# bnbowman/pbccs

Hardware: AMD Instinct MI355X
Metric: CCS ZMWs/sec (and GCUPS) at 1/2/4/8 MI355X vs host-CPU ccs (higher is better)
Workload: dtype f64

## Files before the change

### pbccs_amd/csrc/arrow_kernels.hip

```cpp
#include "arrow_device.hpp"
#include "arrow_kernels.hpp"
#include "arrow_score_device.hpp"
#include "coop_chain.hpp"

#include <climits>

namespace pbccs {

__device__ __forceinline__ LaneBand scratch_band(const FillScratch& F, int g, int l, int which)
{
    const long long gm = 2LL * g + which;
    LaneBand m;
    m.range = F.range + gm * F.capCols * 64 + l;
    m.off = F.off + gm * F.capCols * 64 + l;
    m.ls = F.ls + gm * F.capCols * 64 + l;
    m.val = F.val + gm * F.capSlots * 64 + l;
    m.cap = F.capSlots;
    return m;
}

__global__ void __launch_bounds__(64) k_fill(DevBatch B, FillScratch F, const int* __restrict__ reads, int n)
{
    const int t = blockIdx.x * blockDim.x + threadIdx.x;
    if (t >= n) return;
// ... 280 lines not shown
            cnt = (p == 0) ? 8 : 6 + (cur != prev ? 1 : 0);
        }
        int incl = cnt;
        for (int d = 1; d < 64; d <<= 1) {
            const int y = __shfl_up(incl, d, 64);
            if (lane >= d) incl += y;
        }
        if (lane == 63) waveSums[wid] = incl;
        __syncthreads();
        int waveOff = 0;
        for (int w = 0; w < wid; ++w) waveOff += waveSums[w];
        const int excl = carry + waveOff + incl - cnt;
        if (p < L) {
            po[p] = excl;
            int k = excl;
            for (int x = 0; x < 4; ++x)
                if (base_char(x) != cur) out[k++] = mut_code(p, kSub, x);
            for (int x = 0; x < 4; ++x)
                if (base_char(x) != prev) out[k++] = mut_code(p, kIns, x);
            if (cur != prev) out[k++] = mut_code(p, kDel, 0);
        }
        __syncthreads();
        if (threadIdx.x == 255) carry = excl + cnt;
        __syncthreads();
    }
    if (threadIdx.x == 0) po[L] = carry;
}

__device__ __forceinline__ bool read_scores(int ts, int te, int type, int ms, int me)
{
    if (type == kIns) return ts <= me && ms <= te;
    return ts < me && ms < te;
}

struct MidGeom {
    int b0, e0, b1, e1;
    int lb, le;
};

__device__ __forceinline__ MidGeom middle_geometry(const Band& a, const Band& b, int sc, int bc)
{
    MidGeom g;
    const int2 r0 = a.range[sc - 1], r1 = a.range[sc], r2 = a.range[sc + 1], r3 = a.range[sc + 2];
    g.b0 = min(min(r1.x, r0.x), r2.x);
    g.e0 = max(max(r1.y, r0.y), r2.y);
    g.b1 = min(min(r2.x, r1.x), r3.x);
    g.e1 = max(max(r2.y, r1.y), r3.y);
    const int2 q0 = b.range[bc], q1 = b.range[bc + 1];
    g.lb = min(min(g.b0, g.b1), min(q0.x, q1.x));
    g.le = max(max(g.e0, g.e1), max(q0.y, q1.y));
    return g;
}

__device__ __forceinline__ double score_middle(const ScoreCtx& S, int sc, int bc, const MidGeom& g,
                                               const double* __restrict__ av, int2 ar,
                                               const double* __restrict__ bv, int2 br,
                                               const char* __restrict__ rdp, TaskStat& st)
{
    const int I = S.I;
    char t0, t1, t2, t3;
    int x0, x1, x2, x3;
    S.tv.At(sc - 2, t0, x0);
    S.tv.At(sc - 1, t1, x1);
    S.tv.At(sc, t2, x2);
    S.tv.At(sc + 1, t3, x3);
    (void)t0;
    const double* P0 = S.P.P(sc > 1 ? x0 : kCtxZero);
    const double* P1 = S.P.P(x1);
    const double* P2 = S.P.P(x2);
    const double pM0 = P0[kM], pD0 = P0[kD], cB0 = P1[kB], cS0 = P1[kS3];
    const double pM1 = P1[kM], pD1 = P1[kD], cB1 = P2[kB], cS1 = P2[kS3];
    const double lM = P2[kM], lD = P2[kD];
    const double pn = S.P.prNot, p3 = S.P.prThird;

#define PB_ALPHA(i) (((i) >= ar.x && (i) < ar.y) ? av[(i)] : 0.0)
#define PB_BETA(i) (((i) >= br.x && (i) < br.y) ? bv[-(i)] : 0.0)
#define PB_CELL(out, i, rb, curB, nxtB, pM, pD, cB, cS, pd, pl, rawPrev)                    \
    {                                                                                     \
        const double em_ = ((rb) == (curB)) ? pn : p3;                                    \
        double s_ = ((i) > 0) ? (((i) < I) ? (pd) * (pM) * em_ : 0.0) : (rawPrev);        \
        if ((i) > 1 && (i) < I) s_ = s_ + (rawPrev) * (((nxtB) == (rb)) ? (cB) : (cS));   \
        if ((i) != I) s_ = s_ + (pl) * (pD);                                              \
        out = s_;                                                                         \
    }

    double C0 = 0.0;
    {
        double aD = PB_ALPHA(g.b0 - 1), raw = 0.0;
        for (int i = g.b0; i < g.e0; ++i) {
            const double aL = PB_ALPHA(i);
            const char rb = rdp[i - 1];
            double v;
            PB_CELL(v, i, rb, t1, t2, pM0, pD0, cB0, cS0, aD, aL, raw);
            raw = v;
            if (C0 < v) C0 = v;
            aD = aL;
        }
    }
    const bool s0 = (C0 != 0.0 && C0 != 1.0);
    const int u0 = min(g.b0, g.b1), u1 = max(g.e0, g.e1);
    double C1 = 0.0;
    {
        double aD = PB_ALPHA(u0 - 1), raw0 = 0.0, raw1 = 0.0, sc0p = 0.0;
        for (int i = u0; i < u1; ++i) {
            const double aL = PB_ALPHA(i);
            const char rb = rdp[i - 1];
            double v0 = 0.0, v1 = 0.0, sc0 = 0.0;
            if (i >= g.b0 && i < g.e0) {
                PB_CELL(v0, i, rb, t1, t2, pM0, pD0, cB0, cS0, aD, aL, raw0);
                sc0 = s0 ? v0 / C0 : v0;
            }
            if (i >= g.b1 && i < g.e1) {
                PB_CELL(v1, i, rb, t2, t3, pM1, pD1, cB1, cS1, sc0p, sc0, raw1);
                if (C1 < v1) C1 = v1;
            }
            raw0 = v0;
            raw1 = v1;
            sc0p = sc0;
            aD = aL;
        }
    }
    const bool s1 = (C1 != 0.0 && C1 != 1.0);
    double v = 0.0;
    {
        double aD = PB_ALPHA(g.lb - 1), raw0 = 0.0, raw1 = 0.0, sc0p = 0.0;
        double bH = PB_BETA(g.lb);
        for (int i = g.lb; i < g.le; ++i) {
            const double aL = PB_ALPHA(i);
            const double bN = PB_BETA(i + 1);
            const char rb = (i >= 1) ? rdp[i - 1] : (char)0;
            double v0 = 0.0, v1 = 0.0, sc0 = 0.0, sc1 = 0.0;
            if (i >= g.b0 && i < g.e0) {
                PB_CELL(v0, i, rb, t1, t2, pM0, pD0, cB0, cS0, aD, aL, raw0);
                sc0 = s0 ? v0 / C0 : v0;
            }
            if (i >= g.b1 && i < g.e1) {
                PB_CELL(v1, i, rb, t2, t3, pM1, pD1, cB1, cS1, sc0p, sc0, raw1);
                sc1 = s1 ? v1 / C1 : v1;
            }
            if (i < I) {
                const double mprob = lM * ((rdp[i] == t3) ? pn : p3);
                v = v + sc1 * mprob * bN;
            }
            v = v + sc1 * lD * bH;
            raw0 = v0;
            raw1 = v1;
            sc0p = sc0;
            aD = aL;
            bH = bN;
        }
    }
#undef PB_CELL
#undef PB_BETA
#undef PB_ALPHA
    const double E = (0.0 + (s0 ? log(C0) : 0.0)) + (s1 ? log(C1) : 0.0);
    st.cells += (unsigned long long)(max(0, g.e0 - g.b0) + max(0, g.e1 - g.b1) + max(0, g.le - g.lb));
    st.bytes += 8ull * (unsigned long long)(max(0, ar.y - ar.x) + max(0, br.y - br.x)) + 16ull * 6ull;
    return ((log(v) + E) + S.bSuf[bc]) + S.aPre[sc];
}

struct Oriented {
    int os, oe, ld, type;
};

__device__ __forceinline__ Oriented setup_score(const DevBatch& B, int r, int code, ScoreCtx& S)
{
    const int z = B.rZmw[r];
    const int L = B.zLen[z];
    const int ts = B.rTs[r], te = B.rTe[r];
    Oriented o;
    o.type = mut_type(code);
    const int pos = mut_pos(code);
    const int base = mut_base(code);
    const int mEnd = (o.type == kIns) ? pos : pos + 1;
    o.ld = (o.type == kIns) ? 1 : (o.type == kDel ? -1 : 0);
    S.B = &B;
    S.P = params_for(B, z);
    S.rd = B.seqPool + B.rSeqOff[r];
    S.I = B.rLen[r];
    S.Jorig = te - ts;
    S.a = band_alpha(B, r);
    S.b = band_beta(B, r);
    const long long cbase = B.rColBase[r];
    S.aPre = B.aPre + cbase;
    S.bSuf = B.bSuf + cbase;
    S.tv = window_view(B, r);
    if (B.rStrand[r] == kFwd) {
        S.tv.vm = make_virtual(S.tv.T, L, o.type, pos, base_char(base));
        o.os = pos - ts;
        o.oe = mEnd - ts;
    } else {
        S.tv.vm = make_virtual(S.tv.T, L, o.type, L - mEnd, base_char(complement_index(base)));
        o.os = te - mEnd;
        o.oe = te - pos;
    }
    return o;
}

__device__ double score_edge(const ScoreCtx& S, const Oriented& o, const ScoreScratch& scratch, TaskStat& st)
{
    const int J = S.Jorig;
    const bool atBegin = o.os < 3;
    const bool atEnd = o.oe > (J + 1) - 1 - 2;
    if (!atBegin && atEnd) {
        const int sc = o.os - 1;
        const int n = S.tv.Length() - sc + 1;
        return extend_alpha_score<TplView, kMaxExtCols>(S, sc, n, false, 0, 0, st);
    }
    if (atBegin && !atEnd) return extend_beta_score<TplView, kMaxExtCols>(S, o.oe, o.ld, st);
    if (!atBegin && !atEnd) {
        const int sc = (o.type == kDel) ? o.os - 1 : o.os;
        return extend_alpha_score<TplView, kMaxExtCols>(S, sc, 2, true, 1 + o.oe, 1 + o.oe + o.ld, st);
    }
    const int Jv = S.tv.Length();
    const long long ncol = Jv + 1;
    const long long need = ncol * (long long)(S.I + 1) + 4 * ncol + 16;
    const unsigned long long at = atomicAdd(scratch.top, (unsigned long long)need);
    if (at + need > scratch.cap) {
        atomicOr(scratch.overflow, 1);
        return __longlong_as_double(0x7ff8000000000001LL);
    }
    double* base0 = scratch.pool + at;
    Band m;
    m.ls = base0;
    m.range = reinterpret_cast<int2*>(base0 + ncol);
    m.off = reinterpret_cast<int*>(base0 + 2 * ncol);
    m.val = base0 + 4 * ncol;
    m.cap = ncol * (long long)(S.I + 1);
    const long long u = fill_alpha(S.tv, S.rd, S.I, m, (const Band*)nullptr, false, S.P);
    st.cells += (unsigned long long)max(0LL, u);
    st.bytes += 8ull * (unsigned long long)max(0LL, u) + 16ull * (unsigned long long)ncol;
    return log(alpha_at(m, S.I, Jv)) + sum_ls(m, Jv + 1);
}

__device__ __forceinline__ int wave_min(int v)
{
    for (int o = 32; o > 0; o >>= 1) v = min(v, __shfl_xor(v, o, 64));
    return v;
}

__device__ __forceinline__ int wave_max(int v)
{
    for (int o = 32; o > 0; o >>= 1) v = max(v, __shfl_xor(v, o, 64));
    return v;
}

#ifndef PBCCS_SCORE_STAGE
#define PBCCS_SCORE_STAGE 448
#endif
constexpr int kScoreWaves = 4;
constexpr int kStageA = PBCCS_SCORE_STAGE;
constexpr int kStageB = PBCCS_SCORE_STAGE;
constexpr int kStageR = PBCCS_SCORE_STAGE;
struct WaveStage {
    double a[kStageA];
    double b[kStageB];
    char rd[kStageR];
};

#ifndef PBCCS_SCORE_WAVES
#define PBCCS_SCORE_WAVES 5
#endif
#if PBCCS_SCORE_WAVES > 0
#define PBCCS_SCORE_OCC __attribute__((amdgpu_waves_per_eu(PBCCS_SCORE_WAVES)))
#else
#define PBCCS_SCORE_OCC
#endif
__global__ void __launch_bounds__(256) PBCCS_SCORE_OCC k_score(DevBatch B, ScoreWork W, ScoreScratch scratch)
{
    __shared__ long long wt0[kScoreWaves];
    if (PBCCS_WAVE_STAMPS && (threadIdx.x & 63) == 0) wt0[threadIdx.x >> 6] = wave_t0(B.stats);
    __shared__ WaveStage stage[kScoreWaves];
    const int wid = __builtin_amdgcn_readfirstlane(threadIdx.x >> 6);
    const long long wave = (long long)blockIdx.x * kScoreWaves + wid;
    const int lane = threadIdx.x & 63;
    const bool waveLive = wave < W.waveStart[W.nWork];
    int k = 0;
    if (waveLive) {
        int lo = 0, hi = W.nWork;
        while (hi - lo > 1) {
            const int mid = (lo + hi) >> 1;
            if (W.waveStart[mid] <= wave) lo = mid; else hi = mid;
        }
        k = lo;
    }
    const int z = waveLive ? W.zmw[k] : 0;
    const int M = waveLive ? W.nMut[k] : 0;
    const int Mc = (waveLive && W.sel) ? W.nSel[k] : M;
    const int chunks = max(1, (Mc + 63) >> 6);
    const long long local = waveLive ? wave - W.waveStart[k] : 0;
    const int rr = W.readLo + (int)(local / chunks);
    const int mc = (int)(local % chunks) * 64 + lane;
    const int r = waveLive ? B.zReadBegin[z] + rr : 0;
    const bool valid = waveLive && mc < Mc && !(B.rCkpt && B.rCkpt[r] != 0);
    const int m = (valid && W.sel) ? (int)(W.sel[W.selBase[k] + mc] - W.mutStart[k]) : mc;

    int code = 0;
    bool scored = false;
    if (valid) {
        code = W.codes[W.mutBase[k] + m];
        const int type = mut_type(code), pos = mut_pos(code);
        const int me = (type == kIns) ? pos : pos + 1;
        scored = B.rActive[r] && read_scores(B.rTs[r], B.rTe[r], type, pos, me);
    }
    ScoreCtx S;
    Oriented o;
    o.os = o.oe = o.ld = o.type = 0;
    bool middle = false;
    int sc = 0, bc = 0;
    MidGeom g;
    g.b0 = g.e0 = g.b1 = g.e1 = g.lb = g.le = 0;
    if (scored) {
        o = setup_score(B, r, code, S);
        const int J = S.Jorig;
        middle = !(o.os < 3) && !(o.oe > J - 2);
        if (middle) {
            sc = (o.type == kDel) ? o.os - 1 : o.os;
            bc = 1 + o.oe;
            g = middle_geometry(S.a, S.b, sc, bc);
        }
    }
    const int aLo = wave_min(middle ? sc - 1 : INT_MAX), aHi = wave_max(middle ? sc - 1 : -1);
    const int bLo = wave_min(middle ? bc : INT_MAX), bHi = wave_max(middle ? bc : -1);
    const int rLo = wave_min(middle ? g.lb - 1 : INT_MAX), rHi = wave_max(middle ? g.le + 1 : -1);
    WaveStage& ws = stage[wid];
    bool staged = false;
    long long aBase = 0, bBase = 0;
    int rBase = 0;
    if (aHi >= 0) {
        const long long cb = B.rColBase[r];
        const int2 rah = B.aRange[cb + aHi];
        const int offLo = B.aOff[cb + aLo], offHi = B.aOff[cb + aHi];
        const int spanA = offHi + (rah.y - rah.x) - offLo;
        const int2 rbl = B.bRange[cb + bLo];
        const int boLo = B.bOff[cb + bLo], boHi = B.bOff[cb + bHi];
        const int spanB = boLo + (rbl.y - rbl.x) - boHi;
        const int I = B.rLen[r];
        const int r0 = max(0, rLo), r1 = min(I, rHi);
        const int spanR = r1 - r0;
        staged = spanA <= kStageA && spanB <= kStageB && spanR <= kStageR;
        if (staged) {
            const double* ga = B.valPool + B.rValA[r] + offLo;
            const double* gb = B.valPool + B.rValB[r] + boHi;
            const char* gr = B.seqPool + B.rSeqOff[r] + r0;
            for (int q = lane; q < spanA; q += 64) ws.a[q] = ga[q];
            for (int q = lane; q < spanB; q += 64) ws.b[q] = gb[q];
            for (int q = lane; q < spanR; q += 64) ws.rd[q] = gr[q];
            aBase = offLo;
            bBase = boHi;
            rBase = r0;
        }
    }
    __syncthreads();

    TaskStat st;
    double d = 0.0;
    if (scored) {
        if (middle) {
            const int2 ar = S.a.range[sc - 1];
            const int2 br = S.b.range[bc];
            const int ao = S.a.off[sc - 1], bo = S.b.off[bc];
            double score;
            if (staged) {
                const double* av = ws.a + (ao - aBase) - ar.x;
                const double* bv = ws.b + (bo - bBase) + (br.y - 1);
                const char* rdp = ws.rd - rBase;
                score = score_middle(S, sc, bc, g, av, ar, bv, br, rdp, st);
            } else {
                const double* av = S.a.val + ao - ar.x;
                const double* bv = S.b.val + bo + (br.y - 1);
                score = score_middle(S, sc, bc, g, av, ar, bv, br, S.rd, st);
            }
            d = score - B.rBaseline[r];
        } else {
            const int slot = atomicAdd(W.edgeCount, 1);
            if (slot < W.edgeCap) {
                W.edgeList[3 * slot + 0] = k;
                W.edgeList[3 * slot + 1] = rr;
                W.edgeList[3 * slot + 2] = m;
            } else {
                atomicOr(scratch.overflow, 2);
            }
        }
    }
    if (valid && !(scored && !middle)) W.delta[W.deltaBase[k] + (long long)rr * M + m] = d;
    if (B.stats) {
        unsigned long long c = st.cells, b = st.bytes;
        for (int q = 32; q > 0; q >>= 1) {
            c += __shfl_xor(c, q, 64);
            b += __shfl_xor(b, q, 64);
        }
        if (lane == 0 && waveLive) {
            atomicAdd(&B.stats[2 * kStatScore], c);
            atomicAdd(&B.stats[2 * kStatScore + 1], b);
        }
        if (PBCCS_WAVE_STAMPS && lane == 0)
            atomicAdd(&B.stats[kWaveScore], (unsigned long long)((long long)__builtin_amdgcn_s_memrealtime() - wt0[wid]));
    }
}


__device__ __forceinline__ void k_score_edge_body(DevBatch B, ScoreWork W, ScoreScratch scratch)
{
    const int t = blockIdx.x * blockDim.x + threadIdx.x;
    if (t >= *W.edgeCount || t >= W.edgeCap) return;
    const int k = W.edgeList[3 * t + 0], rr = W.edgeList[3 * t + 1], m = W.edgeList[3 * t + 2];
    const int z = W.zmw[k];
    const int M = W.nMut[k];
    const int r = B.zReadBegin[z] + rr;
    const int code = W.codes[W.mutBase[k] + m];
    ScoreCtx S;
    const Oriented o = setup_score(B, r, code, S);
    TaskStat st;
    const double d = score_edge(S, o, scratch, st) - B.rBaseline[r];
    W.delta[W.deltaBase[k] + (long long)rr * M + m] = d;
    if (B.stats) {
        atomicAdd(&B.stats[2 * kStatScore], st.cells);
        atomicAdd(&B.stats[2 * kStatScore + 1], st.bytes);
    }
}
__global__ void __launch_bounds__(64) k_score_edge(DevBatch B, ScoreWork W, ScoreScratch scratch)
{
    k_score_edge_body(B, W, scratch);
}

constexpr int kCkptCols = 3 * kCkptMaxK + 8;

struct ReplayRead {
    const char* rd;
    const char* T;
    int I, J, L, start;
    const double* ctx;
    double prNot, prThird;
    __device__ __forceinline__ int TB(int idx) const
    {
        const int g = start + idx;
        return (idx <= J && g < L) ? coop::base_code(T[g]) : coop::kBaseOther;
    }
    __device__ __forceinline__ int TC(int idx) const
    {
        return (start + idx + 1 < L) ? coop::ctx_code(TB(idx), TB(idx + 1)) : kCtxZero;
    }
    __device__ __forceinline__ int RB(int i) const { return (i >= 0 && i < I) ? coop::base_code(rd[i]) : 15; }
};
// ... 213 lines not shown
            const bool mine = pending && ja / K == q;
            const int aHi = wave_max(mine ? ja : -1);
            const int jbLo = wave_min(mine ? bc : INT_MAX), jbHi = wave_max(mine ? bc : -1);
            const int ckA = q * K;
            int ckB = jbHi;
            while (!ckpt_col_b(ckB, J, K)) ++ckB;
            const int nA = aHi - ckA + 1, nB = ckB - jbLo + 1;
            long long need = 0;
            if (nA + nB <= kCkptCols) {
                long long hsum = 0;
                for (int c = lane; c < nA + nB; c += 64) {
                    const int2 rg = c < nA ? aR[ckA + c] : bR[ckB - (c - nA)];
                    hsum += max(0, rg.y - rg.x);
                }
                for (int w = 32; w > 0; w >>= 1) hsum += __shfl_xor(hsum, w, 64);
                need = hsum;
            }
            if (nA + nB > kCkptCols || need > C.slotCap) {
                if (lane == 0) atomicMax(C.need, nA + nB > kCkptCols ? kCkptBadGeometry : (unsigned long long)need);
                pending = pending && !mine;
                continue;
            }
            if (lane == 0) {
                int o2 = 0;
                for (int c = 0; c < nA + nB; ++c) {
                    const int2 rg = c < nA ? aR[ckA + c] : bR[ckB - (c - nA)];
                    sOff[c] = o2;
                    o2 += max(0, rg.y - rg.x);
                }
            }
            __syncthreads();
            {
                const int2 r0 = aR[ckA];
                const double* src = aV + aO[ckA];
                for (int i = lane; i < r0.y - r0.x; i += 64) slot[sOff[0] + i] = src[i];
                for (int j = ckA + 1; j <= aHi; ++j) {
                    const int2 pr = aR[j - 1], rg = aR[j];
                    __builtin_amdgcn_fence(__ATOMIC_ACQ_REL, "workgroup");
                    replay_alpha(X, j, slot + sOff[j - 1 - ckA], pr.x, pr.y, slot + sOff[j - ckA], rg.x, rg.y);
                }
            }
            {
                const int2 r0 = bR[ckB];
                const double* src = bV + bO[ckB];
                for (int i = lane; i < r0.y - r0.x; i += 64) slot[sOff[nA] + i] = src[i];
                for (int j = ckB - 1; j >= jbLo; --j) {
                    const int2 nr = bR[j + 1], rg = bR[j];
                    __builtin_amdgcn_fence(__ATOMIC_ACQ_REL, "workgroup");
                    replay_beta(X, j, slot + sOff[nA + (ckB - (j + 1))], nr.x, nr.y, slot + sOff[nA + (ckB - j)], rg.x,
                                rg.y);
                }
            }
            __builtin_amdgcn_fence(__ATOMIC_ACQ_REL, "workgroup");
            if (mine) {
                const int2 ar = aR[ja];
                const int2 br = bR[bc];
                const double* av = slot + sOff[ja - ckA] - ar.x;
                const double* bv = slot + sOff[nA + (ckB - bc)] + (br.y - 1);
                const double score = score_middle(S, sc, bc, g, av, ar, bv, br, S.rd, st);
                W.delta[W.deltaBase[k] + (long long)rr * M + m] = score - B.rBaseline[r];
            }
            pending = pending && !mine;
            __syncthreads();
        }
        if (B.stats) {
            unsigned long long c2 = st.cells, b2 = st.bytes;
            for (int w = 32; w > 0; w >>= 1) {
                c2 += __shfl_xor(c2, w, 64);
                b2 += __shfl_xor(b2, w, 64);
            }
            if (lane == 0) {
                atomicAdd(&B.stats[2 * kStatScore], c2);
                atomicAdd(&B.stats[2 * kStatScore + 1], b2);
            }
        }
    }
}
__global__ void __launch_bounds__(64) k_score_ckpt(DevBatch B, ScoreWork W, CkptWork C)
{
    k_score_ckpt_body(B, W, C);
}

__device__ __forceinline__ void k_reduce_body(DevBatch B, ScoreWork W, double fastThr, double* __restrict__ score,
                                                unsigned char* __restrict__ fav)
{
    const long long g = (long long)blockIdx.x * blockDim.x + threadIdx.x;
    if (g >= W.mutStart[W.nWork]) return;
    int lo = 0, hi = W.nWork;
    while (hi - lo > 1) {
        const int mid = (lo + hi) >> 1;
        if (W.mutStart[mid] <= g) lo = mid; else hi = mid;
    }
    const int k = lo;
    const int z = W.zmw[k];
    const int M = W.nMut[k];
    const int m = (int)(g - W.mutStart[k]);
    const int code = W.codes[W.mutBase[k] + m];
    const int type = mut_type(code), pos = mut_pos(code);
    const int me = (type == kIns) ? pos : pos + 1;
    const int rb = B.zReadBegin[z], nr = B.zNReads[z];
    const double* d = W.delta + W.deltaBase[k] + m;
    double sum = 0.0;
    const double e = W.dev ? W.dev[k] : 0.0;
    bool amb = false;
    for (int rr = 0; rr < nr; ++rr) {
        const int r = rb + rr;
        if (B.rActive[r] && read_scores(B.rTs[r], B.rTe[r], type, pos, me)) sum += d[(long long)rr * M];
        if (e > 0.0) amb = amb || fabs(sum - fastThr) <= e + 1e-12 * fabs(fastThr);
        if (sum < fastThr) break;
    }
    score[W.mutBase[k] + m] = sum;
    fav[W.mutBase[k] + m] = (sum > 0.04) ? 1 : 0;
// ... 287 lines not shown
```

### pbccs_amd/csrc/arrow_kernels.hpp

```cpp
#pragma once

#include <hip/hip_runtime.h>

#include "arrow_device.hpp"

namespace pbccs {

struct ScoreWork {
    int nWork = 0;
    const int* zmw = nullptr;
    const int* nMut = nullptr;
    const long long* mutBase = nullptr;
    const long long* deltaBase = nullptr;
    const long long* waveStart = nullptr;
    const long long* mutStart = nullptr;
    const long long* posStart = nullptr;
    const int* codes = nullptr;
    double* delta = nullptr;
    int* edgeList = nullptr;
    int* edgeCount = nullptr;
    int edgeCap = 0;
    int readLo = 0;
    int readHi = 1 << 30;
    const long long* sel = nullptr;
    const long long* selBase = nullptr;
    const int* nSel = nullptr;
    const double* dev = nullptr;
    int* amb = nullptr;
};

constexpr int kCkptMaxK = 32;
constexpr unsigned long long kCkptBadGeometry = 1ull << 62;
struct CkptWork {
    const int2* pairs = nullptr;
    const long long* taskStart = nullptr;
    int nPairs = 0;
    long long nTasks = 0;
    unsigned long long* counter = nullptr;
    double* slots = nullptr;
    long long slotCap = 0;
    int nSlots = 0;
    unsigned long long* need = nullptr;
};

struct ScoreScratch {
    double* pool = nullptr;
    unsigned long long* top = nullptr;
    unsigned long long cap = 0;
    int* overflow = nullptr;
};

struct WideTask {
    int r;
    int type;
    int os, oe;
    int nb;
    int slot;
    unsigned long long bases;
};
constexpr int kWideMaxBases = 7;
constexpr int kWideExtColumns = 8;
constexpr int kWideRefillWidth = 3;
__host__ __device__ inline bool wide_task_refills(int os, int oe, int nb, int J)
{
    return (os < 3 && oe > J - 2) || (nb > oe - os ? nb : oe - os) >= kWideRefillWidth;
}

struct FillScratch {
    double* val = nullptr;
    int2* range = nullptr;
    int* off = nullptr;
    double* ls = nullptr;
    double* pre = nullptr;
    int* usedA = nullptr;
    int* usedB = nullptr;
    long long capSlots = 0;
    int capCols = 0;
    long long* trace = nullptr;
};

struct CoopFill {
// ... 65 lines not shown
```

### pbccs_amd/csrc/engine.hip

```cpp
#include "engine.hpp"
#include "diploid_kernels.hpp"
#include "refine_repeats.hpp"
#include "strand_kernels.hpp"

#include <hipcub/hipcub.hpp>

#include <algorithm>
#include <mutex>
#include <climits>
#include <cmath>
#include <cstdio>
#include <cstdlib>
#include <cstring>
#include <numeric>
#include <set>
#include <stdexcept>
#include <chrono>
#include <unordered_set>

namespace pbccs {

#define PBCCS_HIP(x)                                                         \
    do {                                                                     \
        hipError_t e_ = (x);                                                 \
// ... 321 lines not shown
    if (evJoin) (void)hipEventDestroy(evJoin);
    if (stream2) (void)hipStreamDestroy(stream2);
    if (stream) (void)hipStreamDestroy(stream);
}

size_t Workspace::TrimRetired()
{
    size_t b = 0;
    auto t = [&](auto& v) { b += v.trim(); };
    t(hDesc);
    t(selBase); t(nSel); t(colScratch); t(bump); t(desc); t(seq); t(ckPairs); t(ckStart); t(rBaseline); t(rFlips);
    t(rDev); t(wDev); t(wAmb);
    t(rStatus); t(usedA); t(usedB); t(maxH); t(wZmw); t(wNMut); t(wMutBase); t(wDeltaBase); t(wWaveStart);
    t(wMutStart); t(wPosStart); t(wPosBase); t(wQvBase); t(stats); t(aRange); t(bRange); t(aOff); t(bOff); t(aLs);
    t(bLs); t(aPre); t(bSuf); t(fVal); t(fLs); t(fPre); t(fRange); t(fOff); t(codes); t(posOff); t(qv); t(list);
    t(edge); t(edgeCount); t(ckSlots); t(ckCounter); t(delta); t(score); t(fav); t(scratch); t(scratchTop);
    t(scratchOverflow); t(xStage); t(sel); t(selCount); t(selScore); t(selCode); t(selRank); t(selTmp);
    b += val.trim_fallback();
    return b;
}

void Workspace::EnsureStreams()
{
    if (stream) return;
    PBCCS_HIP(hipStreamCreateWithFlags(&stream, hipStreamNonBlocking));
    PBCCS_HIP(hipStreamCreateWithFlags(&stream2, hipStreamNonBlocking));
    PBCCS_HIP(hipEventCreateWithFlags(&evFork, hipEventDisableTiming));
    PBCCS_HIP(hipEventCreateWithFlags(&evJoin, hipEventDisableTiming));
}

ArrowBatch::ArrowBatch(int device, Workspace* shared, bool ownStreams, bool wsBuffers)
    : device_(device),
      ownWs_(shared ? nullptr : new Workspace()),
      ws_(shared ? shared : ownWs_.get()),
      dSelBase_(ws_->selBase), dNSel_(ws_->nSel), dColScratch_(ws_->colScratch), dBump_(ws_->bump),
      hDesc_(ws_->hDesc), dCkPairs_(ws_->ckPairs), dCkStart_(ws_->ckStart), dRBaseline_(ws_->rBaseline),
      dRDev_(ws_->rDev),
      dRFlips_(ws_->rFlips), dRStatus_(ws_->rStatus), dUsedA_(ws_->usedA), dUsedB_(ws_->usedB), dMaxH_(ws_->maxH),
      dWZmw_(ws_->wZmw), dWNMut_(ws_->wNMut), dWMutBase_(ws_->wMutBase), dWDeltaBase_(ws_->wDeltaBase),
      dWWaveStart_(ws_->wWaveStart), dWMutStart_(ws_->wMutStart), dWPosStart_(ws_->wPosStart),
      dWPosBase_(ws_->wPosBase), dWQvBase_(ws_->wQvBase),
      dARange_(ws_->aRange), dBRange_(ws_->bRange), dAOff_(ws_->aOff), dBOff_(ws_->bOff), dALs_(ws_->aLs),
      dBLs_(ws_->bLs), dAPre_(ws_->aPre), dBSuf_(ws_->bSuf), dVal_(ws_->val), dCodes_(ws_->codes),
      dPosOff_(ws_->posOff), dQv_(ws_->qv), dList_(ws_->list), dEdge_(ws_->edge), dEdgeCount_(ws_->edgeCount),
      dDelta_(ws_->delta), dScore_(ws_->score), dFav_(ws_->fav), dScratch_(ws_->scratch),
      dScratchTop_(ws_->scratchTop), dScratchOverflow_(ws_->scratchOverflow), dStats_(ws_->stats),
      eventPool_(ws_->eventPool), dDesc_(wsBuffers && shared ? ws_->desc : ownDesc_),
      dSeq_(wsBuffers && shared ? ws_->seq : ownSeq_)
{
    PBCCS_HIP(hipSetDevice(device_));
    if (const char* e = std::getenv("PBCCS_INITIAL_BAND_HEIGHT")) initialBandHeight_ = std::max(1, std::atoi(e));
    ckpt_policy(&ckptK_, &ckptMinLen_);
    ckptAll_ = std::min(kCkptMaxK, std::max(0, env_int("PBCCS_CKPT_ALL", 0)));
    if (ownStreams) {
        ownStreams_ = true;
        PBCCS_HIP(hipStreamCreateWithFlags(&stream_, hipStreamNonBlocking));
        static const bool oneStream = env_int("PBCCS_ONE_STREAM", 0) != 0;
        if (oneStream) stream2_ = stream_;
        else PBCCS_HIP(hipStreamCreateWithFlags(&stream2_, hipStreamNonBlocking));
        PBCCS_HIP(hipEventCreateWithFlags(&evFork_, hipEventDisableTiming));
        PBCCS_HIP(hipEventCreateWithFlags(&evJoin_, hipEventDisableTiming));
    } else {
        ws_->EnsureStreams();
        stream_ = ws_->stream;
        stream2_ = ws_->stream2;
        evFork_ = ws_->evFork;
        evJoin_ = ws_->evJoin;
    }
    const StreamScope bound(stream_);
    if (shared && std::getenv("PBCCS_DBG_CLEAR") && std::getenv("PBCCS_DBG_CLEAR")[0] == '1') {
        PBCCS_HIP(hipDeviceSynchronize());
        auto z = [](auto& v) {
            if (v.ptr) PBCCS_HIP(hipMemset(v.ptr, 0, v.cap * sizeof(*v.ptr)));
        };
        Workspace& w = *ws_;
        z(w.selBase); z(w.nSel); z(w.colScratch); z(w.bump); z(w.ckPairs); z(w.ckStart); z(w.rBaseline);
        z(w.rFlips); z(w.rStatus); z(w.usedA); z(w.usedB); z(w.maxH); z(w.wZmw); z(w.wNMut); z(w.wMutBase);
        z(w.wDeltaBase); z(w.wWaveStart); z(w.wMutStart); z(w.wPosStart); z(w.wPosBase); z(w.wQvBase); z(w.stats);
        if (w.hDesc.ptr) std::memset(w.hDesc.ptr, 0, w.hDesc.cap);
        PBCCS_HIP(hipDeviceSynchronize());
    }
    dScratch_.reserve(kInitialScratch, false);
    dScratchTop_.reserve(1, false);
    hSeq_.assign(16, '\0');
    seqTop_ = 16;
    dScratchOverflow_.reserve(1, false);
}

ArrowBatch::~ArrowBatch()
{
    if (stream_) {
        (void)hipStreamSynchronize(stream_);
        (void)hipStreamSynchronize(stream2_);
        for (const Pending& p : pending_) {
            eventPool_.push_back(p.a);
            eventPool_.push_back(p.b);
        }
        if (ownStreams_) {
            (void)hipEventDestroy(evFork_);
            (void)hipEventDestroy(evJoin_);
            if (stream2_ != stream_) (void)hipStreamDestroy(stream2_);
            (void)hipStreamDestroy(stream_);
        }
    }
}

// ... 1046 lines not shown
    rPosStart_.assign(n + 1, 0);
    rDeltaBase_.assign(n, 0);
    std::vector<long long> waveStart(n + 1, 0), posBase(n, 0);
    long long delta = 0, posOffTotal = 0;
    for (int k = 0; k < n; ++k) {
        const HZmw& z = zmws_[zl[k]];
        const long long M = codes ? (long long)(*codes)[k].size() : unique_mutation_count(z.tpl);
        rNMut_[k] = (int)M;
        rMutStart_[k + 1] = rMutStart_[k] + M;
        rDeltaBase_[k] = delta;
        delta += M * z.nReads;
        waveStart[k + 1] = waveStart[k] + (long long)z.nReads * ((M + 63) / 64);
        rPosStart_[k + 1] = rPosStart_[k] + (long long)z.tpl.size();
        posBase[k] = posOffTotal;
        posOffTotal += (long long)z.tpl.size() + 1;
    }
    rTotalMut_ = rMutStart_[n];
    rTotalPos_ = rPosStart_[n];
    rTotalDelta_ = delta;
    std::vector<long long> mutBase(rMutStart_.begin(), rMutStart_.begin() + n);
    upload_packed({xfer_ul(dWZmw_, zl), xfer_ul(dWNMut_, rNMut_), xfer_ul(dWMutBase_, mutBase),
                   xfer_ul(dWDeltaBase_, rDeltaBase_), xfer_ul(dWWaveStart_, waveStart), xfer_ul(dWMutStart_, rMutStart_),
                   xfer_ul(dWPosStart_, rPosStart_), xfer_ul(dWPosBase_, posBase)},
                  ws_->xStage, hXStage_, stream_);
    dCodes_.reserve(std::max<long long>(rTotalMut_, 1), false);
    dScore_.reserve(std::max<long long>(rTotalMut_, 1), false);
    dFav_.reserve(std::max<long long>(rTotalMut_, 1), false);
    dDelta_.reserve(std::max<long long>(rTotalDelta_, 1), false);
    const DevBatch B = View();
    if (codes) {
        std::vector<int> flat;
        flat.reserve(rTotalMut_);
        for (const std::vector<int>& c : *codes) flat.insert(flat.end(), c.begin(), c.end());
        upload(dCodes_, flat, stream_);
        PBCCS_HIP(hipStreamSynchronize(stream_));
    } else {
        dPosOff_.reserve(std::max<long long>(posOffTotal, 1), false);
        Timed(kKEnumerate, [&] {
            launch_enumerate(B, dWZmw_.ptr, n, dWMutBase_.ptr, dWPosBase_.ptr, dCodes_.ptr, dPosOff_.ptr, stream_);
        });
    }
    (void)needPositions;
    ScoreWork W;
    W.nWork = n;
    W.zmw = dWZmw_.ptr;
    W.nMut = dWNMut_.ptr;
    W.mutBase = dWMutBase_.ptr;
    W.deltaBase = dWDeltaBase_.ptr;
    W.waveStart = dWWaveStart_.ptr;
    W.mutStart = dWMutStart_.ptr;
    W.posStart = dWPosStart_.ptr;
    W.codes = dCodes_.ptr;
    W.delta = dDelta_.ptr;
    {
        std::vector<double> dev(n, 0.0);
        bool any = false;
        for (int k = 0; k < n; ++k) {
            const HZmw& z = zmws_[zl[k]];
            for (int q = 0; q < z.nReads; ++q) {
                const HRead& h = reads_[z.readBegin + q];
                if (h.active && h.dev > 0.0) dev[k] += 3.0 * h.dev;
            }
            any = any || dev[k] > 0.0;
        }
        rDevItem_ = dev;
        if (any) {
            upload(ws_->wDev, dev, stream_);
            ws_->wAmb.reserve(std::max(n, 1), false);
            PBCCS_HIP(hipMemsetAsync(ws_->wAmb.ptr, 0, std::max(n, 1) * sizeof(int), stream_));
            W.dev = ws_->wDev.ptr;
            W.amb = ws_->wAmb.ptr;
        }
        rAmbOn_ = any;
    }
    long long edgeCap = 0;
    for (int k = 0; k < n; ++k) edgeCap += 80LL * zmws_[zl[k]].nReads;
    edgeCap = std::min<long long>(std::max<long long>(edgeCap, 64), rTotalDelta_ + 64);
    dEdge_.reserve(3 * edgeCap, false);
    dEdgeCount_.reserve(1, false);
    W.edgeList = dEdge_.ptr;
    W.edgeCount = dEdgeCount_.ptr;
    W.edgeCap = (int)edgeCap;
    bool anyCkpt = false;
    for (int k = 0; k < n && !anyCkpt; ++k) {
        const HZmw& z = zmws_[zl[k]];
        for (int q = 0; q < z.nReads; ++q) anyCkpt = anyCkpt || reads_[z.readBegin + q].ckpt != 0;
    }
    CkptWork ck;
    auto ckpt_tasks = [&](int lo, int hi, const std::vector<int>* nSelH) {
        ck = CkptWork();
        if (!anyCkpt) return;
        std::vector<int2> pairs;
        std::vector<long long> start{0};
        long long maxI = 1;
        int maxK = 1;
        for (int k = 0; k < n; ++k) {
            const HZmw& z = zmws_[zl[k]];
            const long long mc = nSelH ? (*nSelH)[k] : rNMut_[k];
            if (mc <= 0) continue;
            for (int q = std::max(0, lo); q < std::min(hi, z.nReads); ++q) {
                const HRead& h = reads_[z.readBegin + q];
                if (h.ckpt == 0) continue;
                pairs.push_back(make_int2(k, q));
                start.push_back(start.back() + (mc + 63) / 64);
                maxI = std::max<long long>(maxI, (long long)h.seq.size() + 1);
                maxK = std::max(maxK, h.ckpt);
// ... 1023 lines not shown
```

### pbccs_amd/csrc/engine.hpp

```cpp
#pragma once

#include <hip/hip_runtime.h>

#include <algorithm>
#include <cstdint>
#include <limits>
#include <memory>
#include <string>
#include <utility>
#include <vector>

#include "arrow_device.hpp"
#include "arrow_kernels.hpp"
#include "arrow_model.hpp"

namespace pbccs {

struct ArrowOptions {
    double scoreDiff = 12.5;
    double fastScoreThreshold = -12.5;
    double addThreshold = std::numeric_limits<double>::quiet_NaN();
};

struct RefineOptions {
// ... 363 lines not shown

    void EnsureZmwUploaded();
    void DeriveZmws();
    void UploadReads();
    void UploadDescriptors();
    void UploadTemplate(int z);
    void EnsureCapacity(int r);
    bool Relayout(const std::vector<int>& reads);
    DevBatch View() const;
    void TraceSummary(size_t n, int H, long long capSlots);
    void MeanVar(const HZmw& z, int strand, int ts, int te, double* mean, double* var) const;
    template <class F>
    void Timed(KernelKind k, F&& launch, hipStream_t st = nullptr);
    void ResolveEvents();
    void RunRound(const std::vector<int>& zmws, const std::vector<std::vector<int>>* codes, double fastThr,
                  bool needPositions, bool phased = false);

    int device_ = 0;
    std::unique_ptr<Workspace> ownWs_;
    Workspace* ws_;
    hipStream_t stream_ = nullptr;
    bool ownStreams_ = false;
    hipStream_t stream2_ = nullptr;
    hipEvent_t evFork_ = nullptr, evJoin_ = nullptr;
    DevVec<long long>& dSelBase_;
    DevVec<int>& dNSel_;
    DevVec<double>& dColScratch_;
    DevVec<long long> dCoopTrace_[4];
    DevVec<unsigned long long> dFillWork_;
    DevVec<unsigned long long>& dBump_;
    std::vector<HZmw> zmws_;
    std::vector<HRead> reads_;
    long long tplTop_ = 0, seqTop_ = 0, colTop_ = 0, valTop_ = 0;
    int initialBandHeight_ = 16;
    bool descDirty_ = true;
    bool reclaim_ = false;
    size_t seqUploaded_ = 0;

    std::vector<char> hTpl_, hSeq_;
    std::vector<unsigned char> hXStage_;
    DevVec<char> ownDesc_, ownSeq_;
    DevVec<char>& dDesc_;
    DevVec<char>& dSeq_;
    PinnedBuf& hDesc_;
    int *pZFwd_ = nullptr, *pZRev_ = nullptr, *pZLen_ = nullptr, *pZReadBegin_ = nullptr, *pZNReads_ = nullptr;
    double* pZCtx_ = nullptr;
    char* pTpl_ = nullptr;
    long long *pRSeqOff_ = nullptr, *pRColBase_ = nullptr, *pRValA_ = nullptr, *pRValB_ = nullptr, *pRValCap_ = nullptr;
    int *pRLen_ = nullptr, *pRStrand_ = nullptr, *pRTs_ = nullptr, *pRTe_ = nullptr, *pRActive_ = nullptr,
        *pRZmw_ = nullptr, *pRCkpt_ = nullptr;
    DevVec<int2>& dCkPairs_;
    DevVec<long long>& dCkStart_;
    int ckptK_ = 0, ckptMinLen_ = 0, ckptAll_ = 0;
    long long ckSlotCap_ = 0;
    DevVec<double>& dRBaseline_;
    DevVec<double>& dRDev_;
    bool scan_ = false;
    DevVec<int>& dRFlips_, &dRStatus_, &dUsedA_, &dUsedB_, &dMaxH_;
    DevVec<int>& dWZmw_, &dWNMut_;
    DevVec<long long>& dWMutBase_, &dWDeltaBase_, &dWWaveStart_, &dWMutStart_, &dWPosStart_, &dWPosBase_,
        &dWQvBase_;
    DevVec<int2>& dARange_;
    DevVec<int2>& dBRange_;
    DevVec<int>& dAOff_;
    DevVec<int>& dBOff_;
    DevVec<double>& dALs_;
    DevVec<double>& dBLs_;
    DevVec<double>& dAPre_;
    DevVec<double>& dBSuf_;
    VmPool& dVal_;
    DevVec<int>& dCodes_;
    DevVec<int>& dPosOff_;
    DevVec<int>& dQv_;
    DevVec<int>& dList_;
    DevVec<int>& dEdge_;
    DevVec<int>& dEdgeCount_;
    DevVec<double>& dDelta_;
    DevVec<double>& dScore_;
    DevVec<unsigned char>& dFav_;
    DevVec<double>& dScratch_;
    DevVec<unsigned long long>& dScratchTop_;
    DevVec<int>& dScratchOverflow_;
    std::vector<long long> rMutStart_, rPosStart_, rDeltaBase_;
    std::vector<int> rNMut_;
    std::vector<double> rDevItem_;
    bool rAmbOn_ = false;
    long long rTotalMut_ = 0, rTotalPos_ = 0, rTotalDelta_ = 0;
    Counters counters_;
    bool profiling_ = false;
    DevVec<unsigned long long>& dStats_;
    DevVec<long long> dTrace_;
    DevVec<float> dSite_;
    DevVec<WideTask> dWide_;
    DevVec<double> dWideDelta_;
    DevVec<int> dRich_;
    DevVec<double> dStrandD_;
    DevVec<int> dStrandI_;
    int wideRows_ = 64;
    DiploidScratch diploid_;
    struct Pending {
        int kind;
        hipEvent_t a, b;
    };
    std::vector<Pending> pending_;
    std::vector<hipEvent_t>& eventPool_;
    KernelStat stats_[kKernelKinds];
// ... 4 lines not shown
```

Measured before the change: 3552.

## Add branch-light interior fast path to middle scoring and DPP wave reductions

Adds an interior specialization of score_middle, used when every lane of the wave has a middle band that lies strictly inside the read and has non-empty alpha/beta ranges. That path drops the per-cell boundary conditionals, clamps loads instead of bounds-checking them, and prefetches the next alpha, beta and read base one step ahead. It also replaces the shuffle-based wave min/max/sum reductions with DPP row-shift and broadcast sequences plus readlane. An env knob (PBCCS_SCORE_PATH) can turn off staging or the interior path for debugging. The risk is subtle numerical or edge-case divergence from the generic path, and the extra code size and register pressure.

```diff
diff --git a/pbccs_amd/csrc/arrow_kernels.hip b/pbccs_amd/csrc/arrow_kernels.hip
--- a/pbccs_amd/csrc/arrow_kernels.hip
+++ b/pbccs_amd/csrc/arrow_kernels.hip
@@ -356,10 +356,15 @@
     return g;
 }
 
+__device__ __forceinline__ bool middle_interior(const MidGeom& g, int I, int2 ar, int2 br)
+{
+    return g.lb >= 2 && g.le <= I && ar.y > ar.x && br.y > br.x;
+}
+
 __device__ __forceinline__ double score_middle(const ScoreCtx& S, int sc, int bc, const MidGeom& g,
                                                const double* __restrict__ av, int2 ar,
                                                const double* __restrict__ bv, int2 br,
-                                               const char* __restrict__ rdp, TaskStat& st)
+                                               const char* __restrict__ rdp, TaskStat& st, bool interior)
 {
     const int I = S.I;
     char t0, t1, t2, t3;
@@ -377,6 +382,94 @@
     const double lM = P2[kM], lD = P2[kD];
     const double pn = S.P.prNot, p3 = S.P.prThird;
 
+    double C0 = 0.0, C1 = 0.0, v = 0.0;
+    bool s0, s1;
+    if (interior) {
+        const int aLast = ar.y - 1, bLast = br.y - 1, rLast = I - 1;
+#define PB_ALPHA_LD(i) av[min(max((i), ar.x), aLast)]
+#define PB_BETA_LD(i) bv[-min(max((i), br.x), bLast)]
+#define PB_IN_A(i) ((i) >= ar.x && (i) < ar.y)
+#define PB_IN_B(i) ((i) >= br.x && (i) < br.y)
+#define PB_CELL_I(e, n, pM, pD, cB, cS, pd, pl, rawPrev) \
+    ((((pd) * (pM) * ((e) ? pn : p3)) + (rawPrev) * ((n) ? (cB) : (cS))) + (pl) * (pD))
+        {
+            double aD = PB_IN_A(g.b0 - 1) ? PB_ALPHA_LD(g.b0 - 1) : 0.0, raw = 0.0;
+            double aN = PB_ALPHA_LD(g.b0);
+            char rbN = rdp[min(g.b0, I) - 1];
+            for (int i = g.b0; i < g.e0; ++i) {
+                const double aL = PB_IN_A(i) ? aN : 0.0;
+                const char rb = rbN;
+                aN = PB_ALPHA_LD(i + 1);
+                rbN = rdp[min(i, rLast)];
+                const double c = PB_CELL_I(rb == t1, t2 == rb, pM0, pD0, cB0, cS0, aD, aL, raw);
+                raw = c;
+                if (C0 < c) C0 = c;
+                aD = aL;
+            }
+        }
+        s0 = (C0 != 0.0 && C0 != 1.0);
+        const int u0 = min(g.b0, g.b1), u1 = max(g.e0, g.e1);
+        {
+            double aD = PB_IN_A(u0 - 1) ? PB_ALPHA_LD(u0 - 1) : 0.0, raw0 = 0.0, raw1 = 0.0, sc0p = 0.0;
+            double aN = PB_ALPHA_LD(u0);
+            char rbN = rdp[min(u0, I) - 1];
+            for (int i = u0; i < u1; ++i) {
+                const double aL = PB_IN_A(i) ? aN : 0.0;
+                const char rb = rbN;
+                aN = PB_ALPHA_LD(i + 1);
+                rbN = rdp[min(i, rLast)];
+                const bool in0 = i >= g.b0 && i < g.e0, in1 = i >= g.b1 && i < g.e1;
+                const bool e2 = rb == t2;
+                const double c0 = PB_CELL_I(rb == t1, e2, pM0, pD0, cB0, cS0, aD, aL, raw0);
+                const double v0 = in0 ? c0 : 0.0;
+                const double sc0 = in0 ? (s0 ? c0 / C0 : c0) : 0.0;
+                const double c1 = PB_CELL_I(e2, t3 == rb, pM1, pD1, cB1, cS1, sc0p, sc0, raw1);
+                const double v1 = in1 ? c1 : 0.0;
+                if (C1 < v1) C1 = v1;
+                raw0 = v0;
+                raw1 = v1;
+                sc0p = sc0;
+                aD = aL;
+            }
+        }
+        s1 = (C1 != 0.0 && C1 != 1.0);
+        {
+            double aD = PB_IN_A(g.lb - 1) ? PB_ALPHA_LD(g.lb - 1) : 0.0, raw0 = 0.0, raw1 = 0.0, sc0p = 0.0;
+            double bH = PB_IN_B(g.lb) ? PB_BETA_LD(g.lb) : 0.0;
+            double aN = PB_ALPHA_LD(g.lb), bNn = PB_BETA_LD(g.lb + 1);
+            char rb = rdp[min(g.lb, I) - 1], rbN = rdp[min(g.lb, rLast)];
+            for (int i = g.lb; i < g.le; ++i) {
+                const double aL = PB_IN_A(i) ? aN : 0.0;
+                const double bN = PB_IN_B(i + 1) ? bNn : 0.0;
+                const char rl = rbN;
+                aN = PB_ALPHA_LD(i + 1);
+                bNn = PB_BETA_LD(i + 2);
+                rbN = rdp[min(i + 1, rLast)];
+                const bool in0 = i >= g.b0 && i < g.e0, in1 = i >= g.b1 && i < g.e1;
+                const bool e2 = rb == t2;
+                const double c0 = PB_CELL_I(rb == t1, e2, pM0, pD0, cB0, cS0, aD, aL, raw0);
+                const double v0 = in0 ? c0 : 0.0;
+                const double sc0 = in0 ? (s0 ? c0 / C0 : c0) : 0.0;
+                const double c1 = PB_CELL_I(e2, t3 == rb, pM1, pD1, cB1, cS1, sc0p, sc0, raw1);
+                const double v1 = in1 ? c1 : 0.0;
+                const double sc1 = in1 ? (s1 ? c1 / C1 : c1) : 0.0;
+                const double mprob = lM * ((rl == t3) ? pn : p3);
+                v = v + sc1 * mprob * bN;
+                v = v + sc1 * lD * bH;
+                raw0 = v0;
+                raw1 = v1;
+                sc0p = sc0;
+                aD = aL;
+                bH = bN;
+                rb = rl;
+            }
+        }
+#undef PB_CELL_I
+#undef PB_IN_B
+#undef PB_IN_A
+#undef PB_BETA_LD
+#undef PB_ALPHA_LD
+    } else {
 #define PB_ALPHA(i) (((i) >= ar.x && (i) < ar.y) ? av[(i)] : 0.0)
 #define PB_BETA(i) (((i) >= br.x && (i) < br.y) ? bv[-(i)] : 0.0)
 #define PB_CELL(out, i, rb, curB, nxtB, pM, pD, cB, cS, pd, pl, rawPrev)                    \
@@ -388,7 +481,6 @@
         out = s_;                                                                         \
     }
 
-    double C0 = 0.0;
     {
         double aD = PB_ALPHA(g.b0 - 1), raw = 0.0;
         for (int i = g.b0; i < g.e0; ++i) {
@@ -401,9 +493,8 @@
             aD = aL;
         }
     }
-    const bool s0 = (C0 != 0.0 && C0 != 1.0);
+    s0 = (C0 != 0.0 && C0 != 1.0);
     const int u0 = min(g.b0, g.b1), u1 = max(g.e0, g.e1);
-    double C1 = 0.0;
     {
         double aD = PB_ALPHA(u0 - 1), raw0 = 0.0, raw1 = 0.0, sc0p = 0.0;
         for (int i = u0; i < u1; ++i) {
@@ -424,8 +515,7 @@
             aD = aL;
         }
     }
-    const bool s1 = (C1 != 0.0 && C1 != 1.0);
-    double v = 0.0;
+    s1 = (C1 != 0.0 && C1 != 1.0);
     {
         double aD = PB_ALPHA(g.lb - 1), raw0 = 0.0, raw1 = 0.0, sc0p = 0.0;
         double bH = PB_BETA(g.lb);
@@ -457,6 +547,7 @@
 #undef PB_CELL
 #undef PB_BETA
 #undef PB_ALPHA
+    }
     const double E = (0.0 + (s0 ? log(C0) : 0.0)) + (s1 ? log(C1) : 0.0);
     st.cells += (unsigned long long)(max(0, g.e0 - g.b0) + max(0, g.e1 - g.b1) + max(0, g.le - g.lb));
     st.bytes += 8ull * (unsigned long long)(max(0, ar.y - ar.x) + max(0, br.y - br.x)) + 16ull * 6ull;
@@ -549,6 +640,57 @@
     return v;
 }
 
+template <int kCtrl, int kRows = 0xf>
+__device__ __forceinline__ int dpp_or_self(int v)
+{
+    return __builtin_amdgcn_update_dpp(v, v, kCtrl, kRows, 0xf, false);
+}
+constexpr int kDppRowShr1 = 0x111, kDppRowShr2 = 0x112, kDppRowShr4 = 0x114, kDppRowShr8 = 0x118;
+constexpr int kDppRowBcast15 = 0x142, kDppRowBcast31 = 0x143;
+
+__device__ __forceinline__ int wave_min_full(int v)
+{
+    v = min(v, dpp_or_self<kDppRowShr1>(v));
+    v = min(v, dpp_or_self<kDppRowShr2>(v));
+    v = min(v, dpp_or_self<kDppRowShr4>(v));
+    v = min(v, dpp_or_self<kDppRowShr8>(v));
+    v = min(v, dpp_or_self<kDppRowBcast15, 0xa>(v));
+    v = min(v, dpp_or_self<kDppRowBcast31, 0xc>(v));
+    return __builtin_amdgcn_readlane(v, 63);
+}
+
+__device__ __forceinline__ int wave_max_full(int v)
+{
+    v = max(v, dpp_or_self<kDppRowShr1>(v));
+    v = max(v, dpp_or_self<kDppRowShr2>(v));
+    v = max(v, dpp_or_self<kDppRowShr4>(v));
+    v = max(v, dpp_or_self<kDppRowShr8>(v));
+    v = max(v, dpp_or_self<kDppRowBcast15, 0xa>(v));
+    v = max(v, dpp_or_self<kDppRowBcast31, 0xc>(v));
+    return __builtin_amdgcn_readlane(v, 63);
+}
+
+template <int kCtrl, int kRows = 0xf>
+__device__ __forceinline__ unsigned long long dpp_or_zero(unsigned long long v)
+{
+    const unsigned lo = (unsigned)__builtin_amdgcn_update_dpp(0, (int)(unsigned)v, kCtrl, kRows, 0xf, false);
+    const unsigned hi = (unsigned)__builtin_amdgcn_update_dpp(0, (int)(unsigned)(v >> 32), kCtrl, kRows, 0xf, false);
+    return ((unsigned long long)hi << 32) | lo;
+}
+
+__device__ __forceinline__ unsigned long long wave_sum_full(unsigned long long v)
+{
+    v += dpp_or_zero<kDppRowShr1>(v);
+    v += dpp_or_zero<kDppRowShr2>(v);
+    v += dpp_or_zero<kDppRowShr4>(v);
+    v += dpp_or_zero<kDppRowShr8>(v);
+    v += dpp_or_zero<kDppRowBcast15, 0xa>(v);
+    v += dpp_or_zero<kDppRowBcast31, 0xc>(v);
+    const unsigned lo = (unsigned)__builtin_amdgcn_readlane((int)(unsigned)v, 63);
+    const unsigned hi = (unsigned)__builtin_amdgcn_readlane((int)(unsigned)(v >> 32), 63);
+    return ((unsigned long long)hi << 32) | lo;
+}
+
 #ifndef PBCCS_SCORE_STAGE
 #define PBCCS_SCORE_STAGE 448
 #endif
@@ -614,6 +756,7 @@
     int sc = 0, bc = 0;
     MidGeom g;
     g.b0 = g.e0 = g.b1 = g.e1 = g.lb = g.le = 0;
+    bool generic = false;
     if (scored) {
         o = setup_score(B, r, code, S);
         const int J = S.Jorig;
@@ -622,11 +765,13 @@
             sc = (o.type == kDel) ? o.os - 1 : o.os;
             bc = 1 + o.oe;
             g = middle_geometry(S.a, S.b, sc, bc);
-        }
-    }
-    const int aLo = wave_min(middle ? sc - 1 : INT_MAX), aHi = wave_max(middle ? sc - 1 : -1);
-    const int bLo = wave_min(middle ? bc : INT_MAX), bHi = wave_max(middle ? bc : -1);
-    const int rLo = wave_min(middle ? g.lb - 1 : INT_MAX), rHi = wave_max(middle ? g.le + 1 : -1);
+            generic = !middle_interior(g, S.I, S.a.range[sc - 1], S.b.range[bc]);
+        }
+    }
+    const bool interior = !(W.scorePath & 2) && __ballot(generic) == 0;
+    const int aLo = wave_min_full(middle ? sc - 1 : INT_MAX), aHi = wave_max_full(middle ? sc - 1 : -1);
+    const int bLo = wave_min_full(middle ? bc : INT_MAX), bHi = wave_max_full(middle ? bc : -1);
+    const int rLo = wave_min_full(middle ? g.lb - 1 : INT_MAX), rHi = wave_max_full(middle ? g.le + 1 : -1);
     WaveStage& ws = stage[wid];
     bool staged = false;
     long long aBase = 0, bBase = 0;
@@ -642,7 +787,7 @@
         const int I = B.rLen[r];
         const int r0 = max(0, rLo), r1 = min(I, rHi);
         const int spanR = r1 - r0;
-        staged = spanA <= kStageA && spanB <= kStageB && spanR <= kStageR;
+        staged = !(W.scorePath & 1) && spanA <= kStageA && spanB <= kStageB && spanR <= kStageR;
         if (staged) {
             const double* ga = B.valPool + B.rValA[r] + offLo;
             const double* gb = B.valPool + B.rValB[r] + boHi;
@@ -669,11 +814,11 @@
                 const double* av = ws.a + (ao - aBase) - ar.x;
                 const double* bv = ws.b + (bo - bBase) + (br.y - 1);
                 const char* rdp = ws.rd - rBase;
-                score = score_middle(S, sc, bc, g, av, ar, bv, br, rdp, st);
+                score = score_middle(S, sc, bc, g, av, ar, bv, br, rdp, st, interior);
             } else {
                 const double* av = S.a.val + ao - ar.x;
                 const double* bv = S.b.val + bo + (br.y - 1);
-                score = score_middle(S, sc, bc, g, av, ar, bv, br, S.rd, st);
+                score = score_middle(S, sc, bc, g, av, ar, bv, br, S.rd, st, interior);
             }
             d = score - B.rBaseline[r];
         } else {
@@ -689,11 +834,7 @@
     }
     if (valid && !(scored && !middle)) W.delta[W.deltaBase[k] + (long long)rr * M + m] = d;
     if (B.stats) {
-        unsigned long long c = st.cells, b = st.bytes;
-        for (int q = 32; q > 0; q >>= 1) {
-            c += __shfl_xor(c, q, 64);
-            b += __shfl_xor(b, q, 64);
-        }
+        const unsigned long long c = wave_sum_full(st.cells), b = wave_sum_full(st.bytes);
         if (lane == 0 && waveLive) {
             atomicAdd(&B.stats[2 * kStatScore], c);
             atomicAdd(&B.stats[2 * kStatScore + 1], b);
@@ -1013,12 +1154,18 @@
                 }
             }
             __builtin_amdgcn_fence(__ATOMIC_ACQ_REL, "workgroup");
+            int2 ar = make_int2(0, 0), br = make_int2(0, 0);
+            bool generic = false;
             if (mine) {
-                const int2 ar = aR[ja];
-                const int2 br = bR[bc];
+                ar = aR[ja];
+                br = bR[bc];
+                generic = !middle_interior(g, X.I, ar, br);
+            }
+            const bool interior = !(W.scorePath & 2) && __ballot(generic) == 0;
+            if (mine) {
                 const double* av = slot + sOff[ja - ckA] - ar.x;
                 const double* bv = slot + sOff[nA + (ckB - bc)] + (br.y - 1);
-                const double score = score_middle(S, sc, bc, g, av, ar, bv, br, S.rd, st);
+                const double score = score_middle(S, sc, bc, g, av, ar, bv, br, S.rd, st, interior);
                 W.delta[W.deltaBase[k] + (long long)rr * M + m] = score - B.rBaseline[r];
             }
             pending = pending && !mine;
diff --git a/pbccs_amd/csrc/arrow_kernels.hpp b/pbccs_amd/csrc/arrow_kernels.hpp
--- a/pbccs_amd/csrc/arrow_kernels.hpp
+++ b/pbccs_amd/csrc/arrow_kernels.hpp
@@ -27,6 +27,7 @@
     const int* nSel = nullptr;
     const double* dev = nullptr;
     int* amb = nullptr;
+    int scorePath = 0;
 };
 
 constexpr int kCkptMaxK = 32;
diff --git a/pbccs_amd/csrc/engine.hip b/pbccs_amd/csrc/engine.hip
--- a/pbccs_amd/csrc/engine.hip
+++ b/pbccs_amd/csrc/engine.hip
@@ -397,6 +397,7 @@
     if (const char* e = std::getenv("PBCCS_INITIAL_BAND_HEIGHT")) initialBandHeight_ = std::max(1, std::atoi(e));
     ckpt_policy(&ckptK_, &ckptMinLen_);
     ckptAll_ = std::min(kCkptMaxK, std::max(0, env_int("PBCCS_CKPT_ALL", 0)));
+    scorePath_ = env_int("PBCCS_SCORE_PATH", 0) & 3;
     if (ownStreams) {
         ownStreams_ = true;
         PBCCS_HIP(hipStreamCreateWithFlags(&stream_, hipStreamNonBlocking));
@@ -1549,6 +1550,7 @@
     W.posStart = dWPosStart_.ptr;
     W.codes = dCodes_.ptr;
     W.delta = dDelta_.ptr;
+    W.scorePath = scorePath_;
     {
         std::vector<double> dev(n, 0.0);
         bool any = false;
diff --git a/pbccs_amd/csrc/engine.hpp b/pbccs_amd/csrc/engine.hpp
--- a/pbccs_amd/csrc/engine.hpp
+++ b/pbccs_amd/csrc/engine.hpp
@@ -439,6 +439,7 @@
     DevVec<int2>& dCkPairs_;
     DevVec<long long>& dCkStart_;
     int ckptK_ = 0, ckptMinLen_ = 0, ckptAll_ = 0;
+    int scorePath_ = 0;
     long long ckSlotCap_ = 0;
     DevVec<double>& dRBaseline_;
     DevVec<double>& dRDev_;
```

New measurement: 3509. 1.2% lower.
